# tqch/ddpm-torch

Measured on AMD Instinct MI355X. Metric: training imgs/s/GPU + 1000-step DDPM samples/s, CIFAR-10 UNet @1/2/4/8 MI355X, higher is better.
Workload: dtype bf16; 1 GPU; configs/cifar10.json UNet (35.7M params), full Trainer.step, B=128 per GPU, 32x32, T=1000, dropout 0.1, Adam+clip+EMA; global_batch=128, rccl_ranks=1, parallelism=dp1

## Files before the change

### ddpm-torch_amd/csrc/elementwise.hip

```cpp
#include "common.h"
#include <stdlib.h>
#include <math.h>

static inline int grid_for(long long n, int block = 256, int cap = 256 * 16) {
    long long g = (n + block - 1) / block;
    if (g > cap) g = cap;
    if (g < 1) g = 1;
    return (int)g;
}

__global__ void temb_kernel(const long long* __restrict__ t, const float* __restrict__ freqs, float* __restrict__ out, int B, int dim) {
    const int half = dim / 2;
    for (int i = blockIdx.x * blockDim.x + threadIdx.x; i < B * dim; i += gridDim.x * blockDim.x) {
        const int b = i / dim, j = i - b * dim;
        float v = 0.f;
        if (j < 2 * half) {
            const float arg = __fmul_rn((float)t[b], freqs[j < half ? j : j - half]);
            v = j < half ? sinf(arg) : cosf(arg);
        }
        out[i] = v;
    }
}
extern "C" int ddpm_timestep_embedding(const long long* t, const float* freqs, float* out, int B, int dim, void* stream) {
    if (!t || !out || !freqs) return DDPM_ERR_NULL;
    if (B <= 0 || dim < 4) return DDPM_ERR_SHAPE;
    hipLaunchKernelGGL(temb_kernel, dim3(grid_for((long long)B * dim)), dim3(256), 0, (hipStream_t)stream, t, freqs, out, B, dim);
    return check_launch();
}

template <typename T>
__global__ void nchw_to_nhwc_kernel(const float* __restrict__ x, T* __restrict__ y, int B, int C, int HW, int Cp) {
    const long long n = (long long)B * HW * Cp;
    for (long long i = (long long)blockIdx.x * blockDim.x + threadIdx.x; i < n; i += (long long)gridDim.x * blockDim.x) {
        const int c = (int)(i % Cp);
        const long long bp = i / Cp;
        const int p = (int)(bp % HW);
        const long long b = bp / HW;
        Elem<T>::st(y + i, c < C ? x[(b * C + c) * HW + p] : 0.f);
    }
}
extern "C" int ddpm_nchw_to_nhwc(const float* x, void* y, int B, int C, int HW, int Cp, int dtype, void* stream) {
    if (!x || !y) return DDPM_ERR_NULL;
    if (B <= 0 || C <= 0 || HW <= 0 || Cp < C) return DDPM_ERR_SHAPE;
    const int g = grid_for((long long)B * HW * Cp);
    if (dtype == DDPM_BF16) hipLaunchKernelGGL(nchw_to_nhwc_kernel<bf16_t>, dim3(g), dim3(256), 0, (hipStream_t)stream, x, (bf16_t*)y, B, C, HW, Cp);
    else if (dtype == DDPM_F32) hipLaunchKernelGGL(nchw_to_nhwc_kernel<float>, dim3(g), dim3(256), 0, (hipStream_t)stream, x, (float*)y, B, C, HW, Cp);
    else return DDPM_ERR_DTYPE;
    return check_launch();
}

template <typename T>
__global__ void pack_weight_kernel(const float* __restrict__ w, T* __restrict__ wf, T* __restrict__ wd, int N, int C, int R, int S, int Cp, int Np) {
    const int RS = R * S;
    if (wf) {
        const long long n = (long long)N * RS * Cp;
        for (long long i = (long long)blockIdx.x * blockDim.x + threadIdx.x; i < n; i += (long long)gridDim.x * blockDim.x) {
            const int c = (int)(i % Cp); const long long r1 = i / Cp;
            const int tap = (int)(r1 % RS); const int nn = (int)(r1 / RS);
            Elem<T>::st(wf + i, c < C ? w[((long long)nn * C + c) * RS + tap] : 0.f);
        }
    }
    if (wd) {
        const long long n = (long long)C * RS * Np;
        for (long long i = (long long)blockIdx.x * blockDim.x + threadIdx.x; i < n; i += (long long)gridDim.x * blockDim.x) {
            const int nn = (int)(i % Np); const long long r1 = i / Np;
            const int tap = (int)(r1 % RS); const int c = (int)(r1 / RS);
            Elem<T>::st(wd + i, nn < N ? w[((long long)nn * C + c) * RS + (RS - 1 - tap)] : 0.f);
        }
    }
}
extern "C" int ddpm_pack_weight(const float* w, void* wf, void* wd, int N, int C, int R, int S, int Cp, int Np, int dtype, void* stream) {
    if (!w || (!wf && !wd)) return DDPM_ERR_NULL;
    if (Cp < C || Np < N) return DDPM_ERR_SHAPE;
    const long long big = (long long)(Cp > C ? Cp : C) * R * S * (Np > N ? Np : N);
    const int g = grid_for(big);
    if (dtype == DDPM_BF16) hipLaunchKernelGGL(pack_weight_kernel<bf16_t>, dim3(g), dim3(256), 0, (hipStream_t)stream, w, (bf16_t*)wf, (bf16_t*)wd, N, C, R, S, Cp, Np);
    else if (dtype == DDPM_F32) hipLaunchKernelGGL(pack_weight_kernel<float>, dim3(g), dim3(256), 0, (hipStream_t)stream, w, (float*)wf, (float*)wd, N, C, R, S, Cp, Np);
    else return DDPM_ERR_DTYPE;
    return check_launch();
}

constexpr int PK_T = 32;
template <typename T> __device__ __forceinline__ void pk_store2(T* p, float a, float b);
template <> __device__ __forceinline__ void pk_store2<bf16_t>(bf16_t* p, float a, float b) { *reinterpret_cast<unsigned*>(p) = pack_bf2(a, b); }
template <> __device__ __forceinline__ void pk_store2<float>(float* p, float a, float b) { *reinterpret_cast<float2*>(p) = make_float2(a, b); }

template <typename T, int RS>
__device__ __forceinline__ void pack_tensor(const float* __restrict__ w, T* __restrict__ wf, T* __restrict__ wd, int N, int C, int Cp, int Np, bool up_dgrad,
                                            float* tile) {
    constexpr int pitch = PK_T * RS + 1;
    const int tiles_c = (Cp + PK_T - 1) / PK_T, tiles_n = (Np + PK_T - 1) / PK_T;
    const int tid = threadIdx.x;
    const bool vec_ok = ((long long)C * RS) % 4 == 0 && (((unsigned long long)w) & 15) == 0;
    for (int t = blockIdx.x; t < tiles_c * tiles_n; t += gridDim.x) {
        const int n0 = (t / tiles_c) * PK_T, c0 = (t % tiles_c) * PK_T;
        const int cw = min(PK_T, C - c0);
        __syncthreads();
        constexpr int V = PK_T * RS / 4, KV = PK_T * V / 256;
        static_assert(PK_T * V % 256 == 0, "whole vectors per thread");
        if (cw == PK_T && vec_ok) {
            float4 xv[KV];
#pragma unroll
            for (int k = 0; k < KV; ++k) {
                const int i = tid + 256 * k, nl = i / V, v = i - nl * V;
                xv[k] = n0 + nl < N ? *reinterpret_cast<const float4*>(w + ((long long)(n0 + nl) * C + c0) * RS + 4 * v) : make_float4(0.f, 0.f, 0.f, 0.f);
            }
#pragma unroll
            for (int k = 0; k < KV; ++k) {
                const int i = tid + 256 * k, nl = i / V, v = i - nl * V;
                float* t4 = tile + nl * pitch + 4 * v;
                t4[0] = xv[k].x; t4[1] = xv[k].y; t4[2] = xv[k].z; t4[3] = xv[k].w;
            }
        } else {
            for (int i = tid; i < PK_T * PK_T * RS; i += 256) {
                const int nl = i / (PK_T * RS), rem = i - nl * (PK_T * RS);
                const bool ok = n0 + nl < N && rem < cw * RS;
                tile[nl * pitch + rem] = ok ? w[((long long)(n0 + nl) * C + c0) * RS + rem] : 0.f;
            }
        }
        __syncthreads();
        constexpr bool BF = sizeof(T) == 2;
        if (wf) {
            if constexpr (BF) {
                for (int i = tid; i < PK_T * RS * (PK_T / 8); i += 256) {
                    const int cl = (i % (PK_T / 8)) * 8, r1 = i / (PK_T / 8), tap = r1 % RS, nl = r1 / RS;
                    if (n0 + nl < N && c0 + cl < Cp) {
                        const float* t8 = tile + nl * pitch + cl * RS + tap;
                        u32x4 o;
                        o.x = pack_bf2(t8[0], t8[RS]); o.y = pack_bf2(t8[2 * RS], t8[3 * RS]); o.z = pack_bf2(t8[4 * RS], t8[5 * RS]); o.w = pack_bf2(t8[6 * RS], t8[7 * RS]);
                        *reinterpret_cast<u32x4*>(wf + ((long long)(n0 + nl) * RS + tap) * Cp + c0 + cl) = o;
                    }
                }
            } else {
                for (int i = tid; i < PK_T * RS * (PK_T / 2); i += 256) {
                    const int cl = (i % (PK_T / 2)) * 2, r1 = i / (PK_T / 2), tap = r1 % RS, nl = r1 / RS;
                    if (n0 + nl < N && c0 + cl < Cp)
                        pk_store2<T>(wf + ((long long)(n0 + nl) * RS + tap) * Cp + c0 + cl, tile[nl * pitch + cl * RS + tap], tile[nl * pitch + (cl + 1) * RS + tap]);
                }
            }
        }
        if constexpr (RS == 9) {
            if (wd && up_dgrad) {
                for (int i = tid; i < PK_T * 16 * (PK_T / 2); i += 256) {
                    const int nl = (i % (PK_T / 2)) * 2, r1 = i / (PK_T / 2), tap = r1 % 16, cl = r1 / 16;
                    if (c0 + cl >= C || n0 + nl >= Np) continue;
                    const int P = tap >> 2, Q = tap & 3;
                    float acc0 = 0.f, acc1 = 0.f;
#pragma unroll
                    for (int a = 0; a < 2; ++a)
#pragma unroll
                        for (int b2 = 0; b2 < 2; ++b2) {
                            const int r = P - a, s2 = Q - b2;
                            if (r >= 0 && r < 3 && s2 >= 0 && s2 < 3) {
                                acc0 += tile[nl * pitch + cl * 9 + (8 - (r * 3 + s2))];
                                acc1 += tile[(nl + 1) * pitch + cl * 9 + (8 - (r * 3 + s2))];
                            }
                        }
                    pk_store2<T>(wd + ((long long)(c0 + cl) * 16 + tap) * Np + n0 + nl, acc0, acc1);
                }
                continue;
            }
        }
        if (wd) {
            if constexpr (BF) {
                for (int i = tid; i < PK_T * RS * (PK_T / 8); i += 256) {
                    const int nl = (i % (PK_T / 8)) * 8, r1 = i / (PK_T / 8), tap = r1 % RS, cl = r1 / RS;
                    if (c0 + cl < C && n0 + nl < Np) {
                        const float* t8 = tile + nl * pitch + cl * RS + (RS - 1 - tap);
                        u32x4 o;
                        o.x = pack_bf2(t8[0], t8[pitch]); o.y = pack_bf2(t8[2 * pitch], t8[3 * pitch]); o.z = pack_bf2(t8[4 * pitch], t8[5 * pitch]);
                        o.w = pack_bf2(t8[6 * pitch], t8[7 * pitch]);
                        *reinterpret_cast<u32x4*>(wd + ((long long)(c0 + cl) * RS + tap) * Np + n0 + nl) = o;
                    }
                }
            } else {
                for (int i = tid; i < PK_T * RS * (PK_T / 2); i += 256) {
                    const int nl = (i % (PK_T / 2)) * 2, r1 = i / (PK_T / 2), tap = r1 % RS, cl = r1 / RS;
                    if (c0 + cl < C && n0 + nl < Np)
                        pk_store2<T>(wd + ((long long)(c0 + cl) * RS + tap) * Np + n0 + nl, tile[nl * pitch + cl * RS + (RS - 1 - tap)],
                                     tile[(nl + 1) * pitch + cl * RS + (RS - 1 - tap)]);
                }
            }
        }
    }
}
template <typename T>
__global__ __launch_bounds__(256)
void pack_weight_multi_kernel(const long long* __restrict__ descs) {
    const long long* d = descs + 8 * (long long)blockIdx.y;
    const float* w = reinterpret_cast<const float*>(d[0]);
    T* wf = reinterpret_cast<T*>(d[1]);
    T* wd = reinterpret_cast<T*>(d[2]);
    const int N = (int)d[3], C = (int)d[4], R = (int)d[5] & 0xff, Cp = (int)d[6], Np = (int)d[7];
    const bool up_dgrad = ((int)d[5] & 0x100) != 0;
    __shared__ float tile[PK_T * (PK_T * 9 + 1)];
    if (R == 3) pack_tensor<T, 9>(w, wf, wd, N, C, Cp, Np, up_dgrad, tile);
    else if (R == 1) pack_tensor<T, 1>(w, wf, wd, N, C, Cp, Np, false, tile);
    else if (R == 2) pack_tensor<T, 4>(w, wf, wd, N, C, Cp, Np, false, tile);
}
extern "C" int ddpm_pack_weight_multi(const long long* descs, int n_tensors, int dtype, void* stream) {
    if (!descs) return DDPM_ERR_NULL;
    if (n_tensors <= 0) return DDPM_OK;
    constexpr int pk_blocks = 256;
    if (dtype == DDPM_BF16) hipLaunchKernelGGL(pack_weight_multi_kernel<bf16_t>, dim3(pk_blocks, n_tensors), dim3(256), 0, (hipStream_t)stream, descs);
    else if (dtype == DDPM_F32) hipLaunchKernelGGL(pack_weight_multi_kernel<float>, dim3(pk_blocks, n_tensors), dim3(256), 0, (hipStream_t)stream, descs);
    else return DDPM_ERR_DTYPE;
    return check_launch();
}

__global__ __launch_bounds__(256) void wgrad_unpack_kernel(const float* __restrict__ gpack, float* __restrict__ gflat, const long long* __restrict__ descs, float scale,
                                                            float* __restrict__ sumsq) {
    __shared__ float sh[4];
    const long long* d = descs + 5 * (long long)blockIdx.y;
    const float* src = gpack + d[0];
    float* dst = gflat + d[1];
    const unsigned C = (unsigned)d[3], RS = (unsigned)d[4];
    const unsigned total = (unsigned)(d[2] * C * RS);
    float acc = 0.f;
    if (RS == 1) {
        for (unsigned i = blockIdx.x * blockDim.x + threadIdx.x; i < total; i += gridDim.x * blockDim.x) {
            const float v = src[i] * scale;
            dst[i] = v; acc += v * v;
        }
    } else if (RS == 9 && C % 64 == 0) {
        __shared__ float slab[4][64 * 9];
        const unsigned lane = threadIdx.x & 63, wave = threadIdx.x >> 6, ctiles = C / 64, items = (unsigned)d[2] * ctiles;
        float* mine = slab[wave];
        for (unsigned it = blockIdx.x * 4 + wave; it < items; it += gridDim.x * 4) {
            const unsigned n = it / ctiles, c0 = (it - n * ctiles) * 64;
            float v[9];
#pragma unroll
            for (int tap = 0; tap < 9; ++tap) v[tap] = src[((unsigned long long)n * 9 + tap) * C + c0 + lane] * scale;
#pragma unroll
            for (int tap = 0; tap < 9; ++tap) { mine[lane * 9 + tap] = v[tap]; acc += v[tap] * v[tap]; }
            __builtin_amdgcn_wave_barrier();
            float* out = dst + ((unsigned long long)n * C + c0) * 9;
#pragma unroll
            for (int k = 0; k < 9; ++k) out[k * 64 + lane] = mine[k * 64 + lane];
            __builtin_amdgcn_wave_barrier();
        }
    } else {
        for (unsigned i = blockIdx.x * blockDim.x + threadIdx.x; i < total; i += gridDim.x * blockDim.x) {
            const unsigned nc = i / RS, tap = i - nc * RS;
            const unsigned n = nc / C, c = nc - n * C;
            const float v = src[((unsigned long long)n * RS + tap) * C + c] * scale;
            dst[i] = v; acc += v * v;
        }
    }
    if (sumsq) {
        acc = wave_sum(acc);
        if ((threadIdx.x & 63) == 0) sh[threadIdx.x >> 6] = acc;
        __syncthreads();
        if (threadIdx.x == 0) sumsq[blockIdx.y * gridDim.x + blockIdx.x] = (sh[0] + sh[1]) + (sh[2] + sh[3]);
    }
}
extern "C" int ddpm_wgrad_unpack(const float* gpack, float* gflat, const long long* descs, int n_tensors, float scale, void* stream) {
    if (!gpack || !gflat || !descs) return DDPM_ERR_NULL;
    if (n_tensors <= 0) return DDPM_OK;
    hipLaunchKernelGGL(wgrad_unpack_kernel, dim3(64, n_tensors), dim3(256), 0, (hipStream_t)stream, gpack, gflat, descs, scale, (float*)nullptr);
    return check_launch();
}
extern "C" int ddpm_wgrad_unpack_sumsq(const float* gpack, float* gflat, const long long* descs, int n_tensors, float scale, float* total_sq,
                                       long long total_sq_floats, void* stream) {
    if (!gpack || !gflat || !descs || !total_sq) return DDPM_ERR_NULL;
    if (n_tensors <= 0) return DDPM_OK;
    if (total_sq_floats < 64 + 64ll * n_tensors) return DDPM_ERR_SHAPE;
    hipLaunchKernelGGL(wgrad_unpack_kernel, dim3(64, n_tensors), dim3(256), 0, (hipStream_t)stream, gpack, gflat, descs, scale, total_sq + 64);
    const int rc = check_launch();
    return rc ? rc : ddpm_sumsq_finish_launch(total_sq + 64, 64 * n_tensors, total_sq, stream);
}

__global__ __launch_bounds__(256) void wgrad_reduce_kernel(const long long* __restrict__ table) {
    const long long* d = table + 5 * (long long)blockIdx.y;
    const float* src = reinterpret_cast<const float*>(d[0]);
    float* dst = reinterpret_cast<float*>(d[1]);
    const long long len = d[2], stride = d[4];
    const int copies = (int)d[3];
    const long long nv = len >> 2;
    for (long long v = (long long)blockIdx.x * blockDim.x + threadIdx.x; v < nv; v += (long long)gridDim.x * blockDim.x) {
        const f32x4* col = reinterpret_cast<const f32x4*>(src) + v;
        const long long sv = stride >> 2;
        f32x4 a = col[0];
        int c = 1;
        for (; c + 8 <= copies; c += 8) {
            f32x4 b[8];
#pragma unroll
            for (int k = 0; k < 8; ++k) b[k] = __builtin_nontemporal_load(col + (long long)(c + k) * sv);
#pragma unroll
            for (int k = 0; k < 8; ++k) a += b[k];
        }
        if (c + 4 <= copies) {
            f32x4 b[4];
#pragma unroll
            for (int k = 0; k < 4; ++k) b[k] = __builtin_nontemporal_load(col + (long long)(c + k) * sv);
#pragma unroll
            for (int k = 0; k < 4; ++k) a += b[k];
            c += 4;
        }
        for (; c < copies; ++c) a += __builtin_nontemporal_load(col + (long long)c * sv);
        reinterpret_cast<f32x4*>(dst)[v] = a;
    }
    if (blockIdx.x == 0 && threadIdx.x < (len & 3)) {
        const long long i = (nv << 2) + threadIdx.x;
        float a = src[i];
        for (int c = 1; c < copies; ++c) a += src[(long long)c * stride + i];
        dst[i] = a;
    }
}
extern "C" int ddpm_wgrad_reduce(const long long* table, int n_tensors, void* stream) {
    if (!table) return DDPM_ERR_NULL;
    if (n_tensors <= 0) return DDPM_OK;
    hipLaunchKernelGGL(wgrad_reduce_kernel, dim3(128, n_tensors), dim3(256), 0, (hipStream_t)stream, table);
    return check_launch();
}

__global__ void mt_gather_kernel(const long long* __restrict__ table) {
    const long long* d = table + 4 * (long long)blockIdx.y;
    const float* a = reinterpret_cast<const float*>(d[0]);
    const float* b = reinterpret_cast<const float*>(d[1]);
    float* dst = reinterpret_cast<float*>(d[2]);
    const long long n = d[3];
    if (((d[0] | d[1] | d[2]) & 15) == 0) {
        const long long nv = n >> 2;
        for (long long i = (long long)blockIdx.x * blockDim.x + threadIdx.x; i < nv; i += (long long)gridDim.x * blockDim.x) {
            f32x4 v = reinterpret_cast<const f32x4*>(a)[i];
            if (b) v += reinterpret_cast<const f32x4*>(b)[i];
            reinterpret_cast<f32x4*>(dst)[i] = v;
        }
        for (long long i = (nv << 2) + (long long)blockIdx.x * blockDim.x + threadIdx.x; i < n; i += (long long)gridDim.x * blockDim.x)
            dst[i] = b ? a[i] + b[i] : a[i];
        return;
    }
    for (long long i = (long long)blockIdx.x * blockDim.x + threadIdx.x; i < n; i += (long long)gridDim.x * blockDim.x)
        dst[i] = b ? a[i] + b[i] : a[i];
}
extern "C" int ddpm_mt_gather_f32(const long long* table, int n_tensors, void* stream) {
    if (!table) return DDPM_ERR_NULL;
    if (n_tensors <= 0) return DDPM_OK;
    hipLaunchKernelGGL(mt_gather_kernel, dim3(32, n_tensors), dim3(256), 0, (hipStream_t)stream, table);
    return check_launch();
}

__global__ void q_sample_kernel(const float* __restrict__ x0, const float* __restrict__ noise, const long long* __restrict__ t,
                                const float* __restrict__ ca, const float* __restrict__ cb, float* __restrict__ xt, int B, int n, int T) {
    const long long tot = (long long)B * n;
    for (long long i = (long long)blockIdx.x * blockDim.x + threadIdx.x; i < tot; i += (long long)gridDim.x * blockDim.x) {
        const int b = (int)(i / n);
        const long long tt = t[b];
        xt[i] = (unsigned long long)tt < (unsigned long long)T ? __fadd_rn(__fmul_rn(ca[tt], x0[i]), __fmul_rn(cb[tt], noise[i])) : __builtin_nanf("");
    }
}
extern "C" int ddpm_q_sample(const float* x0, const float* noise, const long long* t, const float* sqrt_ab, const float* sqrt_1mab,
                             float* xt, int B, int n, int T, void* stream) {
    if (!x0 || !noise || !t || !sqrt_ab || !sqrt_1mab || !xt) return DDPM_ERR_NULL;
    if (B <= 0 || n <= 0 || T <= 0) return DDPM_ERR_SHAPE;
    hipLaunchKernelGGL(q_sample_kernel, dim3(grid_for((long long)B * n)), dim3(256), 0, (hipStream_t)stream, x0, noise, t, sqrt_ab, sqrt_1mab, xt, B, n, T);
    return check_launch();
}

__global__ __launch_bounds__(1024) void mse_fwd_kernel(const float* __restrict__ pred, const float* __restrict__ target, float* __restrict__ loss, int n) {
    __shared__ float sh[16];
    const int b = blockIdx.x;
    const float* p = pred + (long long)b * n;
    const float* t = target + (long long)b * n;
    float acc = 0.f;
    const bool al = ((reinterpret_cast<unsigned long long>(p) | reinterpret_cast<unsigned long long>(t)) & 15) == 0;
    const int nv = al ? n >> 2 : 0;
    int i = threadIdx.x;
    for (; i + 3 * (int)blockDim.x < nv; i += 4 * blockDim.x) {
        f32x4 a[4], c[4];
#pragma unroll
        for (int u = 0; u < 4; ++u) { a[u] = reinterpret_cast<const f32x4*>(t)[i + u * blockDim.x]; c[u] = reinterpret_cast<const f32x4*>(p)[i + u * blockDim.x]; }
#pragma unroll
        for (int u = 0; u < 4; ++u) { const f32x4 d = a[u] - c[u]; acc += (d.x * d.x + d.y * d.y) + (d.z * d.z + d.w * d.w); }
    }
    for (; i < nv; i += blockDim.x) { const f32x4 d = reinterpret_cast<const f32x4*>(t)[i] - reinterpret_cast<const f32x4*>(p)[i]; acc += (d.x * d.x + d.y * d.y) + (d.z * d.z + d.w * d.w); }
    for (int j = (nv << 2) + threadIdx.x; j < n; j += blockDim.x) { const float d = t[j] - p[j]; acc += d * d; }
    acc = wave_sum(acc);
    if ((threadIdx.x & 63) == 0) sh[threadIdx.x >> 6] = acc;
    __syncthreads();
    if (threadIdx.x == 0) {
        float tot = 0.f;
        for (int w = 0; w < (int)(blockDim.x >> 6); ++w) tot += sh[w];
        loss[b] = tot / (float)n;
    }
}
__global__ void mse_bwd_kernel(const float* __restrict__ pred, const float* __restrict__ target, const float* __restrict__ gloss,
                               float* __restrict__ gpred, int B, int n) {
    const long long tot = (long long)B * n;
    const float inv = 2.0f / (float)n;
    for (long long i = (long long)blockIdx.x * blockDim.x + threadIdx.x; i < tot; i += (long long)gridDim.x * blockDim.x) {
        const int b = (int)(i / n);
        gpred[i] = (pred[i] - target[i]) * inv * gloss[b];
    }
}
extern "C" int ddpm_mse_fwd(const float* pred, const float* target, float* loss, int B, int n, void* stream) {
    if (!pred || !target || !loss) return DDPM_ERR_NULL;
    if (B <= 0 || n <= 0) return DDPM_ERR_SHAPE;
    hipLaunchKernelGGL(mse_fwd_kernel, dim3(B), dim3(n >= 16384 ? 1024 : 256), 0, (hipStream_t)stream, pred, target, loss, n);
    return check_launch();
}
extern "C" int ddpm_mse_bwd(const float* pred, const float* target, const float* gloss, float* gpred, int B, int n, void* stream) {
    if (!pred || !target || !gloss || !gpred) return DDPM_ERR_NULL;
    if (B <= 0 || n <= 0) return DDPM_ERR_SHAPE;
    hipLaunchKernelGGL(mse_bwd_kernel, dim3(grid_for((long long)B * n)), dim3(256), 0, (hipStream_t)stream, pred, target, gloss, gpred, B, n);
    return check_launch();
}

struct VlbTables { const float *recip, *recip_m1, *coef1, *coef2, *post_logvar, *model_logvar; };
struct VlbCoef { float recip, recip_m1, c1, c2, lv1, lv2; };
__device__ __forceinline__ float vlb_cdf(float z) {
    return 0.5f * (1.0f + tanhf(0.7978845608028654f * (z + 0.044715f * z * z * z)));
}
__device__ __forceinline__ float vlb_cdf_grad(float z) {
    const float th = tanhf(0.7978845608028654f * (z + 0.044715f * z * z * z));
    return 0.5f * (1.0f - th * th) * 0.7978845608028654f * (1.0f + 3.0f * 0.044715f * z * z);
}
__device__ __forceinline__ void vlb_model_mean(const VlbCoef& k, int mean_type, int clip, float xt, float o, float& mean, float& x0p) {
    if (mean_type == 0) x0p = __fsub_rn(__fmul_rn(k.recip, xt), __fmul_rn(k.recip_m1, o));
    else if (mean_type == 1) x0p = o;
    else x0p = __fsub_rn(__fdiv_rn(o, k.c1), __fmul_rn(__fdiv_rn(k.c2, k.c1), xt));
    if (clip) x0p = x0p != x0p ? x0p : fminf(fmaxf(x0p, -1.f), 1.f);
    mean = mean_type == 2 ? o : __fadd_rn(__fmul_rn(k.c1, x0p), __fmul_rn(k.c2, xt));
}
__global__ __launch_bounds__(256) void vlb_terms_kernel(const float* __restrict__ x0, const float* __restrict__ xt, const float* __restrict__ out,
                                                        const long long* __restrict__ t, VlbTables tb, float* __restrict__ loss,
                                                        float* __restrict__ pred_x0, int n, int mean_type, int clip, int T) {
    __shared__ float sh[4];
    const int b = blockIdx.x;
    const long long tt = t[b];
    const long long base = (long long)b * n;
    if ((unsigned long long)tt >= (unsigned long long)T) {
        if (threadIdx.x == 0) loss[b] = __builtin_nanf("");
        if (pred_x0) for (int i = threadIdx.x; i < n; i += blockDim.x) pred_x0[base + i] = __builtin_nanf("");
        return;
    }
    const VlbCoef k{tb.recip[tt], tb.recip_m1[tt], tb.coef1[tt], tb.coef2[tt], tb.post_logvar[tt], tb.model_logvar[tt]};
    const float dlv = k.lv1 - k.lv2, e_dlv = expf(dlv), inv_var2 = expf(-k.lv2), inv_std = expf(-0.5f * k.lv2);
    float acc = 0.f;
    for (int i = threadIdx.x; i < n; i += blockDim.x) {
        const float x = x0[base + i], xti = xt[base + i];
        float mean, x0p;
        vlb_model_mean(k, mean_type, clip, xti, out[base + i], mean, x0p);
        if (pred_x0) pred_x0[base + i] = x0p;
        float term;
        if (tt > 0) {
            const float m1 = __fadd_rn(__fmul_rn(k.c1, x), __fmul_rn(k.c2, xti)), d = m1 - mean;
            term = 0.5f * ((-1.0f - dlv) + d * d * inv_var2 + e_dlv);
        } else {
            const float xc = x - mean;
            const float cu = x > 0.999f ? 1.0f : vlb_cdf(inv_std * (xc + (1.0f / 255.0f)));
            const float cl = x < -0.999f ? 0.0f : vlb_cdf(inv_std * (xc - (1.0f / 255.0f)));
            term = -logf(fmaxf(cu - cl - 1e-12f, 0.f) + 1e-12f);
        }
        acc += term;
    }
    acc = wave_sum(acc);
    if ((threadIdx.x & 63) == 0) sh[threadIdx.x >> 6] = acc;
    __syncthreads();
    if (threadIdx.x == 0) loss[b] = ((sh[0] + sh[1]) + (sh[2] + sh[3])) / (float)n / 0.6931471805599453f;
}
__global__ void vlb_terms_bwd_kernel(const float* __restrict__ x0, const float* __restrict__ xt, const float* __restrict__ out,
                                     const long long* __restrict__ t, VlbTables tb, const float* __restrict__ gloss, float* __restrict__ gout,
                                     int B, int n, int mean_type, int T) {
    const long long tot = (long long)B * n;
    const float inv = 1.0f / ((float)n * 0.6931471805599453f);
    for (long long i = (long long)blockIdx.x * blockDim.x + threadIdx.x; i < tot; i += (long long)gridDim.x * blockDim.x) {
        const int b = (int)(i / n);
        const long long tt = t[b];
        if ((unsigned long long)tt >= (unsigned long long)T) { gout[i] = __builtin_nanf(""); continue; }
        const VlbCoef k{tb.recip[tt], tb.recip_m1[tt], tb.coef1[tt], tb.coef2[tt], tb.post_logvar[tt], tb.model_logvar[tt]};
        const float x = x0[i], xti = xt[i];
        float mean, x0p;
        vlb_model_mean(k, mean_type, 0, xti, out[i], mean, x0p);
        float dterm_dmean;
        if (tt > 0) {
            const float m1 = __fadd_rn(__fmul_rn(k.c1, x), __fmul_rn(k.c2, xti));
            dterm_dmean = -(m1 - mean) * expf(-k.lv2);
        } else {
            const float inv_std = expf(-0.5f * k.lv2), xc = x - mean;
            const float zu = inv_std * (xc + (1.0f / 255.0f)), zl = inv_std * (xc - (1.0f / 255.0f));
            const float cu = x > 0.999f ? 1.0f : vlb_cdf(zu), cl = x < -0.999f ? 0.0f : vlb_cdf(zl);
            const float p = cu - cl - 1e-12f;
            const float dp = -inv_std * ((x > 0.999f ? 0.f : vlb_cdf_grad(zu)) - (x < -0.999f ? 0.f : vlb_cdf_grad(zl)));
            dterm_dmean = p > 0.f ? -dp / (p + 1e-12f) : 0.f;
        }
        const float dmean_dout = mean_type == 0 ? -k.c1 * k.recip_m1 : (mean_type == 1 ? k.c1 : 1.0f);
        gout[i] = gloss[b] * inv * dterm_dmean * dmean_dout;
    }
}
extern "C" int ddpm_vlb_terms(const float* x_0, const float* x_t, const float* model_out, const long long* t,
                              const float* sqrt_recip_ab, const float* sqrt_recip_m1_ab, const float* post_coef1, const float* post_coef2,
                              const float* post_logvar, const float* model_logvar, float* loss, float* pred_x0,
                              int B, int n, int mean_type, int clip, int T, void* stream) {
    if (!x_0 || !x_t || !model_out || !t || !sqrt_recip_ab || !sqrt_recip_m1_ab || !post_coef1 || !post_coef2 || !post_logvar || !model_logvar || !loss)
        return DDPM_ERR_NULL;
    if (B <= 0 || n <= 0 || T <= 0 || mean_type < 0 || mean_type > 2) return DDPM_ERR_SHAPE;
    VlbTables tb{sqrt_recip_ab, sqrt_recip_m1_ab, post_coef1, post_coef2, post_logvar, model_logvar};
    hipLaunchKernelGGL(vlb_terms_kernel, dim3(B), dim3(256), 0, (hipStream_t)stream, x_0, x_t, model_out, t, tb, loss, pred_x0, n, mean_type, clip, T);
    return check_launch();
}
extern "C" int ddpm_vlb_terms_bwd(const float* x_0, const float* x_t, const float* model_out, const long long* t,
                                  const float* sqrt_recip_ab, const float* sqrt_recip_m1_ab, const float* post_coef1, const float* post_coef2,
                                  const float* post_logvar, const float* model_logvar, const float* gloss, float* gout,
                                  int B, int n, int mean_type, int T, void* stream) {
    if (!x_0 || !x_t || !model_out || !t || !sqrt_recip_ab || !sqrt_recip_m1_ab || !post_coef1 || !post_coef2 || !post_logvar || !model_logvar || !gloss || !gout)
        return DDPM_ERR_NULL;
    if (B <= 0 || n <= 0 || T <= 0 || mean_type < 0 || mean_type > 2) return DDPM_ERR_SHAPE;
    VlbTables tb{sqrt_recip_ab, sqrt_recip_m1_ab, post_coef1, post_coef2, post_logvar, model_logvar};
    hipLaunchKernelGGL(vlb_terms_bwd_kernel, dim3(grid_for((long long)B * n)), dim3(256), 0, (hipStream_t)stream, x_0, x_t, model_out, t, tb, gloss, gout,
                       B, n, mean_type, T);
    return check_launch();
}

struct BpdConst { VlbCoef k; float dlv, e_dlv, inv_var2, inv_std; };
__device__ __forceinline__ BpdConst bpd_const(const VlbTables& tb, long long tt) {
    BpdConst c;
    c.k = VlbCoef{tb.recip[tt], tb.recip_m1[tt], tb.coef1[tt], tb.coef2[tt], tb.post_logvar[tt], tb.model_logvar[tt]};
    c.dlv = c.k.lv1 - c.k.lv2; c.e_dlv = expf(c.dlv); c.inv_var2 = expf(-c.k.lv2); c.inv_std = expf(-0.5f * c.k.lv2);
    return c;
}
__device__ __forceinline__ void bpd_elem(const BpdConst& c, long long tt, int mean_type, int clip, int decoder, float x, float xti, float o,
                                         float& term, float& sq) {
    const VlbCoef& k = c.k;
    float mean, x0p;
    vlb_model_mean(k, mean_type, clip, xti, o, mean, x0p);
    if (tt > 0) {
        const float m1 = __fadd_rn(__fmul_rn(k.c1, x), __fmul_rn(k.c2, xti)), d = m1 - mean;
        term = 0.5f * ((-1.0f - c.dlv) + d * d * c.inv_var2 + c.e_dlv);
    } else if (decoder == 0) {
        const float xc = x - mean;
        const float cu = x > 0.999f ? 1.0f : vlb_cdf(c.inv_std * (xc + (1.0f / 255.0f)));
        const float cl = x < -0.999f ? 0.0f : vlb_cdf(c.inv_std * (xc - (1.0f / 255.0f)));
        term = -logf(fmaxf(cu - cl - 1e-12f, 0.f) + 1e-12f);
    } else {
        const float xc = x - mean;
        term = 0.5f * (xc * xc * c.inv_var2 + 1.8378770664093453f + k.lv2);
    }
    const float e = x0p - x;
    sq = e * e;
}
struct BpdArgs {
    const float *x0, *xt, *out;
    const long long* t;
    VlbTables tb;
    float *losses, *mses;
    int B, n, ld, mean_type, clip, decoder, T;
};
__global__ __launch_bounds__(256) void bpd_terms_wave_kernel(BpdArgs a) {
    const int b = blockIdx.x * 4 + (threadIdx.x >> 6), lane = threadIdx.x & 63;
    if (b >= a.B) return;
    const long long tt = a.t[b];
    if ((unsigned long long)tt >= (unsigned long long)a.T) return;
    const long long base = (long long)b * a.n;
    const BpdConst c = bpd_const(a.tb, tt);
    float acc = 0.f, acc2 = 0.f;
    for (int i = lane; i < a.n; i += 64) {
        float term, sq;
        bpd_elem(c, tt, a.mean_type, a.clip, a.decoder, a.x0[base + i], a.xt[base + i], a.out[base + i], term, sq);
        acc += term; acc2 += sq;
    }
    acc = wave_sum(acc); acc2 = wave_sum(acc2);
    if (lane == 0) {
        a.losses[(long long)b * a.ld + tt] = acc / (float)a.n / 0.6931471805599453f;
        a.mses[(long long)b * a.ld + tt] = acc2 / (float)a.n;
    }
}
template <int THREADS>
__global__ __launch_bounds__(THREADS) void bpd_terms_kernel(BpdArgs a) {
    constexpr int WAVES = THREADS / 64;
    __shared__ float sh[2][WAVES];
    const int b = blockIdx.x;
    const long long tt = a.t[b];
    if ((unsigned long long)tt >= (unsigned long long)a.T) return;
    const long long base = (long long)b * a.n;
    const float *x0 = a.x0 + base, *xt = a.xt + base, *out = a.out + base;
    const BpdConst c = bpd_const(a.tb, tt);
    float acc = 0.f, acc2 = 0.f;
    int nv = 0;
    if (THREADS == 1024) {
        const bool al = ((reinterpret_cast<unsigned long long>(x0) | reinterpret_cast<unsigned long long>(xt) | reinterpret_cast<unsigned long long>(out)) & 15) == 0;
        nv = al ? a.n >> 2 : 0;
        int i = threadIdx.x;
        for (; i + THREADS < nv; i += 2 * THREADS) {
            f32x4 vx[2], vt[2], vo[2];
#pragma unroll
            for (int u = 0; u < 2; ++u) {
                vx[u] = reinterpret_cast<const f32x4*>(x0)[i + u * THREADS];
                vt[u] = reinterpret_cast<const f32x4*>(xt)[i + u * THREADS];
                vo[u] = reinterpret_cast<const f32x4*>(out)[i + u * THREADS];
            }
#pragma unroll
            for (int u = 0; u < 2; ++u)
#pragma unroll
                for (int e = 0; e < 4; ++e) {
                    float term, sq;
                    bpd_elem(c, tt, a.mean_type, a.clip, a.decoder, vx[u][e], vt[u][e], vo[u][e], term, sq);
                    acc += term; acc2 += sq;
                }
        }
        for (; i < nv; i += THREADS) {
            const f32x4 vx = reinterpret_cast<const f32x4*>(x0)[i], vt = reinterpret_cast<const f32x4*>(xt)[i], vo = reinterpret_cast<const f32x4*>(out)[i];
#pragma unroll
            for (int e = 0; e < 4; ++e) {
                float term, sq;
                bpd_elem(c, tt, a.mean_type, a.clip, a.decoder, vx[e], vt[e], vo[e], term, sq);
                acc += term; acc2 += sq;
            }
        }
    }
    for (int i = (nv << 2) + threadIdx.x; i < a.n; i += THREADS) {
        float term, sq;
        bpd_elem(c, tt, a.mean_type, a.clip, a.decoder, x0[i], xt[i], out[i], term, sq);
        acc += term; acc2 += sq;
    }
    acc = wave_sum(acc); acc2 = wave_sum(acc2);
// ... 523 lines not shown
```

Before: 14430 imgs/s.

## Rewrite wgrad reduce as persistent chunked kernel balanced across all tensors

Replaces the 2D grid (128 blocks per tensor) with a persistent grid sized to the CU count. That grid walks a flattened list of 256-element chunks across all tensors, using a shared-memory prefix of per-tensor chunk counts. Each thread sums one scalar column across the copies with a deep 32-way unrolled nontemporal load chain, with tails of 16/8/4/2. The aim is to fix load imbalance between tiny and large tensors and to raise memory-level parallelism. The costs are scalar rather than vector loads, higher register use, and multiple launches when there are more than 256 tensors.

```diff
diff --git a/ddpm-torch_amd/csrc/elementwise.hip b/ddpm-torch_amd/csrc/elementwise.hip
--- a/ddpm-torch_amd/csrc/elementwise.hip
+++ b/ddpm-torch_amd/csrc/elementwise.hip
@@ -270,48 +270,76 @@
     return rc ? rc : ddpm_sumsq_finish_launch(total_sq + 64, 64 * n_tensors, total_sq, stream);
 }
 
-__global__ __launch_bounds__(256) void wgrad_reduce_kernel(const long long* __restrict__ table) {
-    const long long* d = table + 5 * (long long)blockIdx.y;
-    const float* src = reinterpret_cast<const float*>(d[0]);
-    float* dst = reinterpret_cast<float*>(d[1]);
-    const long long len = d[2], stride = d[4];
-    const int copies = (int)d[3];
-    const long long nv = len >> 2;
-    for (long long v = (long long)blockIdx.x * blockDim.x + threadIdx.x; v < nv; v += (long long)gridDim.x * blockDim.x) {
-        const f32x4* col = reinterpret_cast<const f32x4*>(src) + v;
-        const long long sv = stride >> 2;
-        f32x4 a = col[0];
-        int c = 1;
-        for (; c + 8 <= copies; c += 8) {
-            f32x4 b[8];
-#pragma unroll
-            for (int k = 0; k < 8; ++k) b[k] = __builtin_nontemporal_load(col + (long long)(c + k) * sv);
-#pragma unroll
-            for (int k = 0; k < 8; ++k) a += b[k];
-        }
-        if (c + 4 <= copies) {
-            f32x4 b[4];
-#pragma unroll
-            for (int k = 0; k < 4; ++k) b[k] = __builtin_nontemporal_load(col + (long long)(c + k) * sv);
-#pragma unroll
-            for (int k = 0; k < 4; ++k) a += b[k];
-            c += 4;
-        }
-        for (; c < copies; ++c) a += __builtin_nontemporal_load(col + (long long)c * sv);
-        reinterpret_cast<f32x4*>(dst)[v] = a;
-    }
-    if (blockIdx.x == 0 && threadIdx.x < (len & 3)) {
-        const long long i = (nv << 2) + threadIdx.x;
-        float a = src[i];
-        for (int c = 1; c < copies; ++c) a += src[(long long)c * stride + i];
-        dst[i] = a;
+constexpr int WGR_COL = 1;
+constexpr int WGR_U = 32;
+constexpr int WGR_BLOCKS_PER_CU = 8;
+constexpr int WGR_CHUNK = 256 * WGR_COL;
+constexpr int WGR_MAX_ROWS = 256;
+#define WGR_GLOBAL __attribute__((address_space(1)))
+template <int N> struct wgr_vec { typedef float type __attribute__((ext_vector_type(N))); };
+template <> struct wgr_vec<1> { typedef float type; };
+template <int N, typename V> __device__ __forceinline__ void wgr_add(V& a, const WGR_GLOBAL float* p, long long stride, unsigned t) {
+    V b[N];
+#pragma unroll
+    for (int k = 0; k < N; ++k) b[k] = __builtin_nontemporal_load(reinterpret_cast<const WGR_GLOBAL V*>(p + k * stride) + t);
+#pragma unroll
+    for (int k = 0; k < N; ++k) a += b[k];
+}
+template <typename V> __device__ __forceinline__ V wgr_column(const WGR_GLOBAL float* p, long long stride, int copies, unsigned t) {
+    V a = __builtin_nontemporal_load(reinterpret_cast<const WGR_GLOBAL V*>(p) + t);
+    int c = 1;
+    for (; c + WGR_U <= copies; c += WGR_U) wgr_add<WGR_U>(a, p + c * stride, stride, t);
+    if (WGR_U > 16 && c + 16 <= copies) { wgr_add<16>(a, p + c * stride, stride, t); c += 16; }
+    if (WGR_U > 8 && c + 8 <= copies) { wgr_add<8>(a, p + c * stride, stride, t); c += 8; }
+    if (WGR_U > 4 && c + 4 <= copies) { wgr_add<4>(a, p + c * stride, stride, t); c += 4; }
+    if (WGR_U > 2 && c + 2 <= copies) { wgr_add<2>(a, p + c * stride, stride, t); c += 2; }
+    for (; c < copies; ++c) wgr_add<1>(a, p + c * stride, stride, t);
+    return a;
+}
+__global__ __launch_bounds__(256) void wgrad_reduce_kernel(const long long* __restrict__ table, int n_rows) {
+    typedef typename wgr_vec<WGR_COL>::type V;
+    __shared__ unsigned chunks[WGR_MAX_ROWS];
+    {
+        const long long len = (int)threadIdx.x < n_rows ? table[5 * threadIdx.x + 2] : 0;
+        chunks[threadIdx.x] = len > 0 ? (unsigned)((len + WGR_CHUNK - 1) / WGR_CHUNK) : 0u;
+    }
+    __syncthreads();
+    int row = 0;
+    unsigned long long first = 0;
+    unsigned nc = chunks[0];
+    for (unsigned long long q = blockIdx.x;; q += gridDim.x) {
+        while (q >= first + nc) {
+            first += nc;
+            if (++row >= n_rows) return;
+            nc = chunks[row];
+        }
+        const long long* d = table + 5 * (long long)__builtin_amdgcn_readfirstlane(row);
+        const long long len = d[2], stride = d[4];
+        const int copies = (int)d[3];
+        const long long c0 = (long long)__builtin_amdgcn_readfirstlane((unsigned)(q - first)) * WGR_CHUNK;
+        const WGR_GLOBAL float* src = (const WGR_GLOBAL float*)(unsigned long long)d[0] + c0;
+        WGR_GLOBAL float* dst = (WGR_GLOBAL float*)(unsigned long long)d[1] + c0;
+        const unsigned t = threadIdx.x;
+        if (c0 + (t + 1) * WGR_COL <= len) {
+            reinterpret_cast<WGR_GLOBAL V*>(dst)[t] = wgr_column<V>(src, stride, copies, t);
+        } else {
+#pragma unroll
+            for (int j = 0; j < WGR_COL - 1; ++j)
+                if (c0 + t * WGR_COL + j < len) dst[t * WGR_COL + j] = wgr_column<float>(src, stride, copies, t * WGR_COL + j);
+        }
     }
 }
 extern "C" int ddpm_wgrad_reduce(const long long* table, int n_tensors, void* stream) {
     if (!table) return DDPM_ERR_NULL;
     if (n_tensors <= 0) return DDPM_OK;
-    hipLaunchKernelGGL(wgrad_reduce_kernel, dim3(128, n_tensors), dim3(256), 0, (hipStream_t)stream, table);
-    return check_launch();
+    const int grid = ddpm_cu_budget(256) * WGR_BLOCKS_PER_CU;
+    for (int r0 = 0; r0 < n_tensors; r0 += WGR_MAX_ROWS) {
+        const int n = n_tensors - r0 < WGR_MAX_ROWS ? n_tensors - r0 : WGR_MAX_ROWS;
+        hipLaunchKernelGGL(wgrad_reduce_kernel, dim3(grid), dim3(256), 0, (hipStream_t)stream, table + 5ll * r0, n);
+        const int rc = check_launch();
+        if (rc) return rc;
+    }
+    return DDPM_OK;
 }
 
 __global__ void mt_gather_kernel(const long long* __restrict__ table) {
```

After: 14500 imgs/s, median of 6. About the same (+0.4%).
